# bfGraph/STGraph

Measured on NVIDIA B200. Metric: gcn_fused_aggregation_fwd_bwd_algorithmic_hbm_gbs, higher is better.
Workload: dtype f32

## Files before the change

include/stgraph_b200.h:

```cpp
#ifndef STGRAPH_B200_H_
#define STGRAPH_B200_H_

#include <stddef.h>
#include <stdint.h>

#ifdef __cplusplus
extern "C" {
#endif

#define STG_ABI_VERSION 3

typedef enum StgStatus {
  STG_OK = 0,
  STG_ERR_INVALID_ARGUMENT = -1,
  STG_ERR_CUDA = -2,
  STG_ERR_UNSUPPORTED = -3,
  STG_ERR_WORKSPACE_TOO_SMALL = -4,
  STG_ERR_CAPACITY = -5
} StgStatus;

typedef struct StgCsrView {
  const int32_t* row_offset;
  const int32_t* column_indices;
  const int32_t* eids;
  const int32_t* node_ids;
  int32_t num_nodes;
  int32_t num_edges;
  int32_t eid_base;
  int32_t eids_identity;
  const int32_t* hub_rows;
  const int32_t* hub_count;
  int32_t hub_threshold;
  int32_t hub_capacity;
  int32_t* work_queue;
} StgCsrView;

int stg_abi_version(void);
const char* stg_last_error(void);
int stg_device_info(int device, int32_t* sm_count, int64_t* l2_bytes, int32_t* cc_major, int32_t* cc_minor);

int stg_agg_scaled_sum_f32(const StgCsrView* g, const float* x, int32_t feat,
                           const float* nbr_scale, const float* edge_scale,
                           const float* row_scale, float* out, void* stream);

typedef struct StgEdgeMeta {
  int32_t col;
  float scale;
} StgEdgeMeta;

int stg_csr_pack_edge_meta_f32(const StgCsrView* g, const float* nbr_scale, const float* edge_scale,
                               StgEdgeMeta* meta, void* stream);

int stg_agg_packed_sum_f32(const StgCsrView* g, const StgEdgeMeta* meta, const float* x, int32_t feat,
                           const float* row_scale, float* out, int32_t accumulate, void* stream);

int stg_agg_packed_sum_strided_f32(const StgCsrView* g, const StgEdgeMeta* meta, const float* x, int32_t feat,
                                   int32_t x_ld, const float* row_scale, float* out, int32_t out_ld,
                                   int32_t accumulate, void* stream);

int stg_agg_scaled_sum_accum_f32(const StgCsrView* g, const float* x, int32_t feat, const float* nbr_scale,
                                 const float* edge_scale, const float* row_scale, float* out, void* stream);

int stg_agg_scaled_sum_red_f32(const StgCsrView* g, const float* x, int32_t feat, const float* nbr_scale,
                               const float* edge_scale, const float* row_scale, float* out, void* stream);

int stg_agg_scaled_sum_rows_f32(const StgCsrView* g, const int32_t* out_rows, const float* x, int32_t feat,
                                const float* nbr_scale, const float* edge_scale, const float* row_scale, float* out,
                                int32_t accumulate, void* stream);

int stg_agg_packed_sum_rows_f32(const StgCsrView* g, const StgEdgeMeta* meta, const int32_t* out_rows, const float* x,
                                int32_t feat, const float* row_scale, float* out, int32_t accumulate, void* stream);

#define STG_MAX_PARTS 16
int stg_agg_scaled_sum_parts_f32(const StgCsrView* g, const float* const* x_parts, const int32_t* part_bounds,
                                 int32_t num_parts, int32_t feat, const float* nbr_scale, const float* edge_scale,
                                 const float* row_scale, float* out, void* stream);

int stg_halo_pull_f32(const float* const* x_parts, const int32_t* part_bounds, int32_t num_parts, const int64_t* ids,
                      int64_t n_ids, int32_t feat, float* out, int32_t max_blocks, void* stream);

int stg_halo_push_f32(const float* own, int32_t feat, const int64_t* send_rows, const int32_t* send_peer,
                      const int64_t* send_slot, int64_t n_items, float* const* peer_halo, int32_t num_parts,
                      int32_t max_blocks, void* stream);

int stg_rows_gather_f32(const float* own, int32_t feat, const int64_t* rows, int64_t n, float* buf, int32_t max_blocks,
                        void* stream);
int stg_halo_send_f32(const float* send_buf, int32_t feat, int32_t num_parts, int32_t my_rank, const int64_t* send_off,
                      float* const* peer_dst, void* stream);
int stg_halo_exchange_f32(const float* own, int32_t feat, const int64_t* send_rows, const int64_t* send_off,
                          float* send_buf, float* const* peer_dst, int32_t* const* peer_flags, const int32_t* seq_values,
                          int32_t value, int32_t num_parts, int32_t my_rank, int32_t gather_blocks, void* stream);
int stg_peer_signal(int32_t* const* peer_flags, int32_t num_parts, int32_t my_rank, int32_t value, void* stream);
// ... 136 lines not shown
```

stgraph_b200/_lib.py:

```python
from __future__ import annotations

import ctypes
import os
import subprocess
from ctypes import POINTER, Structure, c_char_p, c_float, c_int32, c_int64, c_size_t, c_void_p

_HERE = os.path.dirname(os.path.abspath(__file__))
LIB_PATH = os.environ.get("STG_B200_LIB") or os.path.join(_HERE, "lib", "libstgraph_b200.so")
CSRC_DIR = os.path.join(_HERE, "csrc")

ABI_VERSION = 3
VM_MAX_TENSORS = 24
VM_MAX_INSTR = 96
VM_MAX_REGS = 48
VM_MAX_ACC = 8


class StgCsrView(Structure):

    _fields_ = [
        ("row_offset", c_void_p),
        ("column_indices", c_void_p),
        ("eids", c_void_p),
        ("node_ids", c_void_p),
# ... 55 lines not shown
                                                  c_void_p, c_void_p], True),
    "stg_agg_scaled_sum_rows_f32": (ctypes.c_int, [_P(StgCsrView), c_void_p, c_void_p, c_int32, c_void_p, c_void_p, c_void_p,
                                                   c_void_p, c_int32, c_void_p], True),
    "stg_csr_pack_edge_meta_f32": (ctypes.c_int, [_P(StgCsrView), c_void_p, c_void_p, c_void_p, c_void_p], True),
    "stg_agg_packed_sum_f32": (ctypes.c_int, [_P(StgCsrView), c_void_p, c_void_p, c_int32, c_void_p, c_void_p, c_int32,
                                              c_void_p], True),
    "stg_agg_packed_sum_strided_f32": (ctypes.c_int, [_P(StgCsrView), c_void_p, c_void_p, c_int32, c_int32, c_void_p,
                                                      c_void_p, c_int32, c_int32, c_void_p], True),
    "stg_halo_push_f32": (ctypes.c_int, [c_void_p, c_int32, c_void_p, c_void_p, c_void_p, c_int64, _P(c_void_p), c_int32,
                                         c_int32, c_void_p], True),
    "stg_agg_packed_sum_rows_f32": (ctypes.c_int, [_P(StgCsrView), c_void_p, c_void_p, c_void_p, c_int32, c_void_p,
                                                   c_void_p, c_int32, c_void_p], True),
    "stg_rows_gather_f32": (ctypes.c_int, [c_void_p, c_int32, c_void_p, c_int64, c_void_p, c_int32, c_void_p], True),
    "stg_halo_send_f32": (ctypes.c_int, [c_void_p, c_int32, c_int32, c_int32, _P(c_int64), _P(c_void_p), c_void_p], True),
    "stg_halo_exchange_f32": (ctypes.c_int, [c_void_p, c_int32, c_void_p, _P(c_int64), c_void_p, _P(c_void_p), _P(c_void_p),
                                              c_void_p, c_int32, c_int32, c_int32, c_int32, c_void_p], True),
    "stg_peer_signal": (ctypes.c_int, [_P(c_void_p), c_int32, c_int32, c_int32, c_void_p], True),
    "stg_peer_wait": (ctypes.c_int, [c_void_p, c_int32, c_int32, c_int32, c_int64, c_void_p, c_void_p], True),
    "stg_agg_scaled_sum_parts_f32": (ctypes.c_int, [_P(StgCsrView), _P(c_void_p), _P(c_int32), c_int32, c_int32, c_void_p,
                                                    c_void_p, c_void_p, c_void_p, c_void_p], True),
    "stg_halo_pull_f32": (ctypes.c_int, [_P(c_void_p), _P(c_int32), c_int32, c_void_p, c_int64, c_int32, c_void_p, c_int32,
                                         c_void_p], True),
    "stg_agg_scaled_sum_f32_host": (ctypes.c_int, [_P(StgCsrView), c_void_p, c_int32, c_void_p, c_void_p, c_void_p,
                                                   c_void_p, c_void_p, c_size_t, c_void_p], True),
    "stg_agg_scaled_sum_f32_host_async": (ctypes.c_int, [_P(StgCsrView), c_void_p, c_int32, c_void_p, c_void_p, c_void_p,
                                                         c_void_p, c_void_p, c_size_t, c_void_p], True),
    "stg_gat_softmax_fwd_f32": (ctypes.c_int, [_P(StgCsrView), c_void_p, c_void_p, c_void_p, c_int32, c_int32,
                                               c_float, c_void_p, c_void_p, c_void_p, c_void_p], True),
    "stg_gat_softmax_bwd_f32": (ctypes.c_int, [_P(StgCsrView), _P(StgCsrView), c_void_p, c_void_p, c_void_p,
                                               c_void_p, c_void_p, c_void_p, c_void_p, c_int32, c_int32, c_float,
                                               c_void_p, c_void_p, c_void_p, c_void_p, c_void_p], True),
    "stg_vm_run_f32": (ctypes.c_int, [_P(StgCsrView), _P(StgVmProgram), _P(c_void_p), c_void_p], True),
    "stg_edge_dot_f32": (ctypes.c_int, [c_void_p, c_int32, c_void_p, c_void_p, c_int64, c_void_p, c_void_p], True),
    "stg_edge_dot_bwd_f32": (ctypes.c_int, [c_void_p, c_int32, c_void_p, c_void_p, c_int64, c_void_p, c_void_p, c_void_p], True),
    "stg_bias_clamp_f32": (ctypes.c_int, [c_void_p, c_void_p, c_int64, c_int32, c_float, c_float, c_void_p], True),
    "stg_clamp_bwd_f32": (ctypes.c_int, [c_void_p, c_void_p, c_void_p, c_int64, c_float, c_float, c_void_p], True),
    "stg_gru_reset_fwd_f32": (ctypes.c_int, [c_void_p, c_void_p, c_void_p, c_int64, c_void_p], True),
    "stg_gru_reset_bwd_f32": (ctypes.c_int, [c_void_p, c_void_p, c_void_p, c_void_p, c_void_p, c_int64, c_void_p], True),
    "stg_gru_update_fwd_f32": (ctypes.c_int, [c_void_p, c_void_p, c_void_p, c_void_p, c_int64, c_void_p], True),
    "stg_gru_update_bwd_f32": (ctypes.c_int, [c_void_p, c_void_p, c_void_p, c_void_p, c_void_p, c_void_p, c_void_p, c_int64,
                                              c_void_p], True),
    "stg_tgcn_reset_fwd_f32": (ctypes.c_int, [c_void_p, c_void_p, c_void_p, c_int64, c_int32, c_void_p], True),
    "stg_tgcn_reset_bwd_f32": (ctypes.c_int, [c_void_p, c_void_p, c_void_p, c_void_p, c_void_p, c_int64, c_int32, c_void_p], True),
    "stg_tgcn_update_fwd_f32": (ctypes.c_int, [c_void_p, c_void_p, c_void_p, c_int64, c_int32, c_void_p], True),
    "stg_tgcn_update_bwd_f32": (ctypes.c_int, [c_void_p, c_void_p, c_void_p, c_void_p, c_void_p, c_int64, c_int32, c_void_p], True),
    "stg_gemm_tn_workspace_bytes": (c_size_t, [c_int64, c_int32, c_int32], False),
    "stg_gemm_tn_f32": (ctypes.c_int, [c_void_p, c_int64, c_void_p, c_int64, c_int64, c_int32, c_int32, c_void_p, c_void_p,
                                       c_void_p, c_size_t, c_void_p], True),
    "stg_csr_build_workspace_bytes": (c_size_t, [c_int64, c_int32], False),
    "stg_csr_build": (ctypes.c_int, [c_void_p, c_void_p, c_int64, c_int32] + [c_void_p] * 12
                      + [c_void_p, c_size_t, c_void_p], True),
    "stg_degree_norm_f32": (ctypes.c_int, [c_void_p, c_int32, c_void_p, c_void_p], True),
    "stg_weighted_row_degree_f32": (ctypes.c_int, [_P(StgCsrView), c_void_p, c_void_p, c_void_p], True),
    "stg_csr_hub_rows": (ctypes.c_int, [c_void_p, c_int32, c_int32, c_void_p, c_int32, c_void_p, c_void_p], True),
    "stg_snapshot_workspace_bytes": (c_size_t, [c_int64], False),
    "stg_snapshot_keys_from_edges": (ctypes.c_int, [c_void_p, c_void_p, c_int64, c_int32, c_void_p, c_void_p, c_void_p,
                                                    c_size_t, c_void_p], True),
    "stg_snapshot_diff": (ctypes.c_int, [c_void_p, c_int64, c_void_p, c_int64, c_void_p, c_void_p, c_void_p, c_size_t,
                                         c_void_p], True),
    "stg_snapshot_apply": (ctypes.c_int, [c_void_p, c_int64, c_void_p, c_int64, c_void_p, c_int64, c_void_p, c_void_p,
                                          c_void_p, c_size_t, c_void_p], True),
    "stg_snapshot_views": (ctypes.c_int, [c_void_p, c_int64, c_int32, c_int32, c_int32] + [c_void_p] * 10
                           + [c_void_p, c_size_t, c_void_p], True),
    "stg_get_array_i32": (ctypes.c_int, [c_void_p, c_int64, c_void_p, c_void_p], True),
}

EXPORTED_SYMBOLS = tuple(_SIGNATURES)

_lib = None


def build(verbose: bool = False) -> str:
    cmd = ["make", "-C", CSRC_DIR, "-j", str(min(8, os.cpu_count() or 1))]
    res = subprocess.run(cmd, stdout=subprocess.PIPE, stderr=subprocess.STDOUT, text=True)
    if verbose or res.returncode != 0:
        print(res.stdout)
    if res.returncode != 0:
        raise RuntimeError("building libstgraph_b200.so failed (see output above)")
    return LIB_PATH


def load():
    global _lib
    if _lib is not None:
        return _lib
    if not os.path.exists(LIB_PATH):
        raise RuntimeError(
            f"{LIB_PATH} is missing: run `python -c 'import __graft_entry__ as g; g.build()'` "
            "(or `make -C stgraph_b200/csrc`). stgraph_b200 has no CPU fallback.")
    lib = ctypes.CDLL(LIB_PATH)
    for name, (restype, argtypes, _) in _SIGNATURES.items():
        fn = getattr(lib, name)
        fn.restype = restype
        fn.argtypes = argtypes
    if lib.stg_abi_version() != ABI_VERSION:
        raise RuntimeError("libstgraph_b200.so ABI version mismatch; rebuild it")
    _lib = lib
    return lib


def call(name: str, *args):
    lib = load()
    rc = getattr(lib, name)(*args)
    if _SIGNATURES[name][2] and rc != 0:
        raise RuntimeError(f"{name} failed ({rc}): {lib.stg_last_error().decode(errors='replace')}")
    return rc
# ... 11 lines not shown
```

stgraph_b200/csrc/agg.cu:

```cuda
#include "common.cuh"

#include <cooperative_groups.h>

#include <algorithm>
#include <cstdlib>

namespace stg {
namespace {

constexpr int kBlockThreads = 256;
constexpr int kHubThreads = 512;

template <int VEC>
__device__ __forceinline__ typename VecT<VEC>::type ld_row(const float* p) {
  using T = typename VecT<VEC>::type;
  return __ldg(reinterpret_cast<const T*>(p));
}
template <int VEC>
__device__ __forceinline__ void st_row(float* p, typename VecT<VEC>::type v) {
  using T = typename VecT<VEC>::type;
  __stcs(reinterpret_cast<T*>(p), v);
}

struct AggParams {
// ... 149 lines not shown
    const int n = min(GROUP, end - base);
    int j = 0;
    for (; j + UNROLL <= n; j += UNROLL) {
      int c[UNROLL];
      float sc[UNROLL];
      T v[UNROLL][NACC];
      fetch_meta(j, c, sc);
#pragma unroll
      for (int u = 0; u < UNROLL; ++u) {
#pragma unroll
        for (int k = 0; k < NACC; ++k) v[u][k] = rows.load(p, c[u], k);
      }
#pragma unroll
      for (int u = 0; u < UNROLL; ++u) {
#pragma unroll
        for (int k = 0; k < NACC; ++k) fma_vec(acc[k], sc[u], v[u][k]);
      }
    }
    if (j < n) {
      int c[UNROLL];
      float sc[UNROLL];
      T v[UNROLL][NACC];
      fetch_meta(j, c, sc);
#pragma unroll
      for (int u = 0; u < UNROLL; ++u) {
#pragma unroll
        for (int k = 0; k < NACC; ++k) {
          if ((j + u) < n) v[u][k] = rows.load(p, c[u], k);
          else zero_vec(v[u][k]);
        }
      }
#pragma unroll
      for (int u = 0; u < UNROLL; ++u) {
#pragma unroll
        for (int k = 0; k < NACC; ++k) fma_vec(acc[k], sc[u], v[u][k]);
      }
    }
    my_c = nx_c;
    my_s = nx_s;
  }
}

template <int VEC, int GROUP, int NACC, int MODE = kPlain>
__device__ __forceinline__ void accumulate_edges(const AggParams& p, int beg, int end, int first_batch,
                                                 int batch_step, int gl, unsigned gmask,
                                                 typename VecT<VEC>::type (&acc)[NACC]) {
  int c;
  float m, s;
  load_col<MODE>(p, beg + first_batch * GROUP, end, gl, c, m);
  load_scale<MODE>(p, beg + first_batch * GROUP, end, gl, c, m, s);
  accumulate_edges<VEC, GROUP, NACC, 0, MODE>(p, beg, end, first_batch, batch_step, gl, gmask, acc, c, s);
}

template <typename T>
__device__ __forceinline__ T shfl_xor_vec(T v, int o);
template <>
__device__ __forceinline__ float shfl_xor_vec<float>(float v, int o) { return __shfl_xor_sync(0xffffffffu, v, o); }
template <>
__device__ __forceinline__ float2 shfl_xor_vec<float2>(float2 v, int o) {
  return make_float2(__shfl_xor_sync(0xffffffffu, v.x, o), __shfl_xor_sync(0xffffffffu, v.y, o));
}
template <>
__device__ __forceinline__ float4 shfl_xor_vec<float4>(float4 v, int o) {
  return make_float4(__shfl_xor_sync(0xffffffffu, v.x, o), __shfl_xor_sync(0xffffffffu, v.y, o),
                     __shfl_xor_sync(0xffffffffu, v.z, o), __shfl_xor_sync(0xffffffffu, v.w, o));
}


__device__ __forceinline__ float4 ldg_row(const float4* p) { return __ldg(p); }

template <int UNROLL, int MODE>
__device__ __forceinline__ void accumulate_edges_pair(const AggParams& p, int beg, int end, int lane, float4& result,
                                                      int my_c, float my_m, float my_s) {
  static_assert(UNROLL % 2 == 0, "two edges per step");
  constexpr int STEPS = UNROLL / 2;
  const int half = lane >> 4;
  const int hl = lane & 15;
  const unsigned ld_bytes = static_cast<unsigned>(p.ld) * 4u;
  const char* base0;
  const char* base1;
  {
    const int last = (p.width - 1) / 4 * 4;
    int o0 = hl * 4, o1 = (hl + 16) * 4;
    if (o0 > last) o0 = last;
    if (o1 > last) o1 = last;
    base0 = reinterpret_cast<const char*>(p.x + o0);
    base1 = reinterpret_cast<const char*>(p.x + o1);
  }
  const bool live1 = (hl + 16) * 4 < p.width;
  auto row0 = [&](int c) { return ldg_row(reinterpret_cast<const float4*>(base0 + static_cast<unsigned long long>(static_cast<unsigned>(c)) * ld_bytes)); };
  auto row1 = [&](int c) {
    float4 v = make_float4(0.f, 0.f, 0.f, 0.f);
    if (live1) v = ldg_row(reinterpret_cast<const float4*>(base1 + static_cast<unsigned long long>(static_cast<unsigned>(c)) * ld_bytes));
    return v;
  };
  float4 acc0 = make_float4(0.f, 0.f, 0.f, 0.f), acc1 = acc0;
  (void)my_m;
  for (int base = beg; base < end; base += 32) {
    int nx_c;
    float nx_m, nx_s;
    load_col<MODE>(p, base + 32, end, lane, nx_c, nx_m);
    load_scale<MODE>(p, base + 32, end, lane, nx_c, nx_m, nx_s);
    const int n = min(32, end - base);
    int j = 0;
    for (; j + UNROLL <= n; j += UNROLL) {
      int c[STEPS];
// ... 188 lines not shown
      if constexpr (PAIR) {
        static_assert(VEC == 4 && GROUP == 32 && NACC == 1, "pair form: one row per warp, float4 lanes");
        accumulate_edges_pair<UNROLL, MODE>(p, beg0, end0, lane, acc[0], c0, 0.f, s0);
      } else {
#pragma unroll
        for (int k = 0; k < NACC; ++k) zero_vec(acc[k]);
        accumulate_edges<VEC, GROUP, NACC, UNROLL, MODE>(p, beg0, end0, 0, 1, gl, gmask, acc, c0, s0);
      }
      write_row<VEC, GROUP, NACC>(p, row0, gl, end0 > beg0, r0, acc, rmw, old);
    }
    slot0 = slot1; row0 = row1; beg0 = beg1; end0 = end1; c0 = c1; s0 = s1; r0 = r1;
    slot1 = slot2; row1 = row2; beg1 = beg2; end1 = end2; c1 = c2; m1 = m2;
    slot2 = slot3; row2 = row3; beg2 = beg3; end2 = end3;
  }
  finish();
}

template <int VEC, int GROUP, int NACC, int MODE, bool PAIR = false>
__global__ void __launch_bounds__(kBlockThreads) agg_rows_kernel(const AggParams p) {
  using T = typename VecT<VEC>::type;
  constexpr int GROUPS_PER_WARP = 32 / GROUP;
  const int lane = threadIdx.x & 31;
  const int gl = lane & (GROUP - 1);
  const unsigned gmask = (GROUP == 32) ? 0xffffffffu : (((1u << GROUP) - 1u) << (lane & ~(GROUP - 1)));
  const int warp = blockIdx.x * (kBlockThreads / 32) + (threadIdx.x >> 5);
  const int row = warp * GROUPS_PER_WARP + lane / GROUP;
  if (row >= p.num_rows) return;
  const int beg = __ldg(p.row_off + row);
  const int end = __ldg(p.row_off + row + 1);
  if (p.hub_threshold > 0 && (end - beg) > p.hub_threshold) return;

  T acc[NACC];
  if constexpr (PAIR) {
    int c;
    float m, s;
    load_col<MODE>(p, beg, end, gl, c, m);
    load_scale<MODE>(p, beg, end, gl, c, m, s);
    accumulate_edges_pair<8, MODE>(p, beg, end, lane, acc[0], c, m, s);
  } else {
#pragma unroll
    for (int k = 0; k < NACC; ++k) zero_vec(acc[k]);
    accumulate_edges<VEC, GROUP, NACC, MODE>(p, beg, end, 0, 1, gl, gmask, acc);
  }

  const int orow = p.out_rows ? __ldg(p.out_rows + row) : row;
  const float r = p.rs ? __ldg(p.rs + orow) : 1.f;
  write_row<VEC, GROUP, NACC>(p, orow, gl, end > beg, r, acc);
  grid_dependency_wait();
}

constexpr int kHubCluster = 8;
constexpr int kClusterRowEdges = 8192;

template <int VEC, int GROUP, int NACC, int MODE>
__global__ void __cluster_dims__(kHubCluster, 1, 1) __launch_bounds__(kHubThreads)
    agg_hub_kernel(const AggParams p) {
  using T = typename VecT<VEC>::type;
  namespace cg = cooperative_groups;
  asm volatile("griddepcontrol.launch_dependents;");
  cg::cluster_group cluster = cg::this_cluster();
  constexpr int GROUPS_PER_WARP = 32 / GROUP;
  constexpr int WARPS = kHubThreads / 32;
  __shared__ T partial[WARPS][GROUP * NACC];
  __shared__ T cta_sum[GROUP * NACC];
  __shared__ int chunk_row[kHubCluster], chunk_beg[kHubCluster], chunk_end[kHubCluster];
  const int lane = threadIdx.x & 31;
  const int wid = threadIdx.x >> 5;
  const int gl = lane & (GROUP - 1);
  const int gidx = lane / GROUP;
  const unsigned gmask = (GROUP == 32) ? 0xffffffffu : (((1u << GROUP) - 1u) << (lane & ~(GROUP - 1)));
  const int crank = static_cast<int>(cluster.block_rank());
  const int cluster_id = blockIdx.x / kHubCluster;
  const int n_clusters = gridDim.x / kHubCluster;
  const int n_hub = min(__ldg(p.hub_count), p.hub_capacity);

  auto cta_partial_sum = [&](int beg, int end, int slot, int slots) {
    T acc[NACC];
#pragma unroll
    for (int k = 0; k < NACC; ++k) zero_vec(acc[k]);
    accumulate_edges<VEC, GROUP, NACC, MODE>(p, beg, end, slot, slots, gl, gmask, acc);
#pragma unroll
    for (int o = GROUP; o < 32; o <<= 1) {
#pragma unroll
      for (int k = 0; k < NACC; ++k) add_vec(acc[k], shfl_xor_vec<T>(acc[k], o));
    }
    if (lane < GROUP) {
#pragma unroll
      for (int k = 0; k < NACC; ++k) partial[wid][k * GROUP + lane] = acc[k];
    }
    __syncthreads();
    if (wid == 0 && lane < GROUP) {
#pragma unroll
      for (int k = 0; k < NACC; ++k) {
        T sum = partial[0][k * GROUP + lane];
        for (int w = 1; w < WARPS; ++w) add_vec(sum, partial[w][k * GROUP + lane]);
        cta_sum[k * GROUP + lane] = sum;
      }
    }
    __syncthreads();
  };
  auto write_hub_row = [&](int row, T (&sum)[NACC]) {
    const int orow = p.out_rows ? __ldg(p.out_rows + row) : row;
    const float r = p.rs ? __ldg(p.rs + orow) : 1.f;
    write_row<VEC, GROUP, NACC>(p, orow, lane, true, r, sum);
  };

  for (int chunk = cluster_id; chunk * kHubCluster < n_hub; chunk += n_clusters) {
    if (threadIdx.x < kHubCluster) {
      const int i = chunk * kHubCluster + threadIdx.x;
      int row = -1, beg = 0, end = 0;
      if (i < n_hub) {
        row = __ldg(p.hub_rows + i);
        beg = __ldg(p.row_off + row);
        end = __ldg(p.row_off + row + 1);
      }
      chunk_row[threadIdx.x] = row;
      chunk_beg[threadIdx.x] = beg;
      chunk_end[threadIdx.x] = end;
    }
    __syncthreads();
    {
      const int row = chunk_row[crank], beg = chunk_beg[crank], end = chunk_end[crank];
      if (row >= 0 && (end - beg) <= kClusterRowEdges) {
        cta_partial_sum(beg, end, wid * GROUPS_PER_WARP + gidx, WARPS * GROUPS_PER_WARP);
        if (wid == 0 && lane < GROUP) {
          T sum[NACC];
#pragma unroll
          for (int k = 0; k < NACC; ++k) sum[k] = cta_sum[k * GROUP + lane];
          write_hub_row(row, sum);
        }
      }
    }
    for (int q = 0; q < kHubCluster; ++q) {
      const int row = chunk_row[q], beg = chunk_beg[q], end = chunk_end[q];
      if (row < 0 || (end - beg) <= kClusterRowEdges) continue;
      cta_partial_sum(beg, end, (crank * WARPS + wid) * GROUPS_PER_WARP + gidx, kHubCluster * WARPS * GROUPS_PER_WARP);
      cluster.sync();
      if (crank == 0 && wid == 0 && lane < GROUP) {
        T sum[NACC];
#pragma unroll
        for (int k = 0; k < NACC; ++k) {
          sum[k] = cta_sum[k * GROUP + lane];
          for (int c = 1; c < kHubCluster; ++c) {
            const T* remote = cluster.map_shared_rank(cta_sum, c);
            add_vec(sum[k], remote[k * GROUP + lane]);
          }
        }
        write_hub_row(row, sum);
      }
      cluster.sync();
    }
    __syncthreads();
  }
}

inline bool pair_mode() {
  static const bool on = [] {
    const char* e = getenv("STG_AGG_PAIR");
    return e == nullptr || e[0] != '0';
  }();
  return on;
}

inline int queue_chunk() {
  static const int v = [] {
    const char* e = getenv("STG_AGG_CHUNK");
    const int c = e ? atoi(e) : 4;
    return c < 0 ? 0 : (c > 4096 ? 4096 : c);
  }();
  return v;
}

inline int hub_grid_mult(int num_edges) {
  static const int v = [] {
    const char* e = getenv("STG_HUB_GRID");
    const int c = e ? atoi(e) : 0;
    return c < 0 ? 0 : (c > 4 ? 4 : c);
  }();
  return v > 0 ? v : (num_edges >= (1 << 24) ? 1 : 2);
}

template <int VEC, int GROUP, int NACC, int MODE>
int launch_agg(const AggParams& p, cudaStream_t stream) {
  constexpr int rows_per_block = (kBlockThreads / 32) * (32 / GROUP);
  const int blocks = (p.num_rows + rows_per_block - 1) / rows_per_block;
  const bool hubs = p.hub_threshold > 0 && p.hub_rows != nullptr;
  const bool overlap = hubs && p.num_edges >= (1 << 18);
  if (hubs) {
    agg_hub_kernel<VEC, GROUP, NACC, MODE><<<hub_grid_mult(p.num_edges) * (sm_count() / kHubCluster) * kHubCluster, kHubThreads, 0, stream>>>(p);
    STG_LAUNCH_CHECK("agg_hub_kernel");
  }
  if (blocks > 0) {
    const bool queue = p.num_rows >= 2 * sm_count() * 4 * (kBlockThreads / 32);
    bool launched = false;
    if constexpr (GROUP == 32 && MODE != kParts) if (queue) {
      launched = true;
      constexpr int MINB = 4;
      constexpr int kRowsPerWarp = 32;
      constexpr int slots_per_block = (kBlockThreads / 32) * kRowsPerWarp;
      const int pblocks = (p.num_rows + slots_per_block - 1) / slots_per_block;
      const bool gq = p.queue != nullptr && queue_chunk() > 0;
      const int gblocks = std::min(sm_count() * MINB, (p.num_rows + 7) / 8);
      if constexpr (VEC == 4 && NACC == 1) {
        if (p.width > 64 && pair_mode()) {
          if (gq) {
            STG_CUDA(launch_overlapped(agg_rows_pipe_kernel<VEC, GROUP, NACC, MINB, 8, MODE, true, true>, gblocks, kBlockThreads,
                                       stream, overlap, p, queue_chunk()));
          } else {
            STG_CUDA(launch_overlapped(agg_rows_pipe_kernel<VEC, GROUP, NACC, MINB, 8, MODE, true>, pblocks, kBlockThreads,
                                       stream, overlap, p, slots_per_block));
          }
          STG_LAUNCH_CHECK("agg_rows_pipe_kernel (pair)");
          return STG_OK;
        }
      }
      if (gq) {
        STG_CUDA(launch_overlapped(agg_rows_pipe_kernel<VEC, GROUP, NACC, MINB, 8 / NACC, MODE, false, true>, gblocks,
                                   kBlockThreads, stream, overlap, p, queue_chunk()));
      } else {
        STG_CUDA(launch_overlapped(agg_rows_pipe_kernel<VEC, GROUP, NACC, MINB, 8 / NACC, MODE>, pblocks, kBlockThreads, stream,
                                   overlap, p, slots_per_block));
      }
    }
    if constexpr (GROUP == 32 && VEC == 4 && NACC == 1 && MODE != kParts) {
      if (!launched && p.width > 64 && pair_mode()) {
        STG_CUDA(launch_overlapped(agg_rows_kernel<VEC, GROUP, NACC, MODE, true>, blocks, kBlockThreads, stream, overlap, p));
        launched = true;
      }
    }
    if (!launched) {
      STG_CUDA(launch_overlapped(agg_rows_kernel<VEC, GROUP, NACC, MODE>, blocks, kBlockThreads, stream, overlap, p));
    }
    STG_LAUNCH_CHECK("agg_rows_kernel");
  }
  return STG_OK;
}

inline bool narrow_vec2() {
  static const bool v = [] {
    const char* e = getenv("STG_AGG_NARROW_VEC2");
    return e ? atoi(e) != 0 : true;
  }();
// ... 65 lines not shown
    al8 = al8 && aligned8(x);
  }
  for (int q = 0; q < nparts; ++q) {
    al16 = al16 && aligned16(parts[q]);
    al8 = al8 && aligned8(parts[q]);
  }
  int vec = 1;
  if (feat % 4 == 0 && p.ld % 4 == 0 && p.ld_out % 4 == 0 && al16) vec = 4;
  else if (feat % 2 == 0 && p.ld % 2 == 0 && p.ld_out % 2 == 0 && al8) vec = 2;
  if (vec == 4 && feat > 32 && feat <= 64 && nparts == 0 && narrow_vec2() && g->work_queue != nullptr &&
      g->num_nodes >= 2 * sm_count() * 4 * (kBlockThreads / 32))
    vec = 2;
  const int chunk = 32 * 4 * vec;
  for (int f0 = 0; f0 < feat; f0 += chunk) {
    p.x = x ? x + f0 : nullptr;
    for (int q = 0; q < nparts; ++q) p.xs[q] = parts[q] + f0;
    p.out = out + f0;
    p.width = min(chunk, feat - f0);
    int rc;
    const int avg_degree = g->num_nodes > 0 ? g->num_edges / g->num_nodes : -1;
    if (nparts > 0) {
      if (vec == 4) rc = dispatch_group<4, kParts>(p, stream, avg_degree);
      else if (vec == 2) rc = dispatch_group<2, kParts>(p, stream, avg_degree);
      else rc = dispatch_group<1, kParts>(p, stream, avg_degree);
    } else if (meta != nullptr) {
      if (vec == 4) rc = dispatch_group<4, kPacked>(p, stream, avg_degree);
      else if (vec == 2) rc = dispatch_group<2, kPacked>(p, stream, avg_degree);
      else rc = dispatch_group<1, kPacked>(p, stream, avg_degree);
    } else {
      if (vec == 4) rc = dispatch_group<4, kPlain>(p, stream, avg_degree);
      else if (vec == 2) rc = dispatch_group<2, kPlain>(p, stream, avg_degree);
      else rc = dispatch_group<1, kPlain>(p, stream, avg_degree);
    }
    if (rc != STG_OK) return rc;
  }
  return STG_OK;
}

}

using namespace stg;

static int validate_view(const StgCsrView* g, bool need_eids) {
  STG_CHECK_ARG(g != nullptr, "graph view is NULL");
  STG_CHECK_ARG(g->num_nodes >= 0 && g->num_edges >= 0, "negative graph size (%d nodes, %d edges)",
                g->num_nodes, g->num_edges);
  STG_CHECK_ARG(g->row_offset != nullptr, "row_offset is NULL");
  STG_CHECK_ARG(g->num_edges == 0 || g->column_indices != nullptr, "column_indices is NULL");
  STG_CHECK_ARG(!need_eids || g->eids_identity || g->num_edges == 0 || g->eids != nullptr,
                "eids is NULL but an edge tensor is indexed by edge id");
  return STG_OK;
}

STG_API int stg_agg_scaled_sum_f32(const StgCsrView* g, const float* x, int32_t feat,
                                      const float* nbr_scale, const float* edge_scale,
                                      const float* row_scale, float* out, void* stream) {
  int rc = validate_view(g, edge_scale != nullptr);
  if (rc != STG_OK) return rc;
  STG_CHECK_ARG(feat > 0, "feat must be positive (got %d)", feat);
  if (g->num_nodes == 0) return STG_OK;
  STG_CHECK_ARG(x != nullptr && out != nullptr, "x / out is NULL");
  STG_CHECK_ARG(x != out, "x and out must not alias");
  return agg_scaled_sum_device(g, x, feat, nbr_scale, edge_scale, row_scale, out, as_stream(stream));
}

static int agg_host_enqueue(const StgCsrView* g, const float* x_host, int32_t feat, const float* nbr_scale_host,
                            const float* edge_scale_host, const float* row_scale_host, float* out_host,
                            void* dev_scratch, size_t dev_scratch_bytes, void* stream, bool synchronize) {
  int rc = validate_view(g, edge_scale_host != nullptr);
  if (rc != STG_OK) return rc;
  STG_CHECK_ARG(feat > 0, "feat must be positive (got %d)", feat);
  if (g->num_nodes == 0) return STG_OK;
  STG_CHECK_ARG(x_host && out_host && dev_scratch, "host buffers / scratch must not be NULL");
  const size_t n = static_cast<size_t>(g->num_nodes), e = static_cast<size_t>(g->num_edges);
  const size_t nf = align_up(n * feat, 4), n4 = align_up(n, 4), e4 = align_up(e, 4);
  const size_t need = (2 * nf + 2 * n4 + e4) * sizeof(float);
  if (dev_scratch_bytes < need) {
    set_error("device scratch too small: %zu bytes given, %zu needed", dev_scratch_bytes, need);
    return STG_ERR_WORKSPACE_TOO_SMALL;
  }
  cudaStream_t s = as_stream(stream);
  float* dx = static_cast<float*>(dev_scratch);
  float* dout = dx + nf;
  float* dns = dout + nf;
  float* drs = dns + n4;
  float* des = drs + n4;
  STG_CUDA(cudaMemcpyAsync(dx, x_host, n * feat * sizeof(float), cudaMemcpyHostToDevice, s));
  if (nbr_scale_host) STG_CUDA(cudaMemcpyAsync(dns, nbr_scale_host, n * sizeof(float), cudaMemcpyHostToDevice, s));
  if (row_scale_host) STG_CUDA(cudaMemcpyAsync(drs, row_scale_host, n * sizeof(float), cudaMemcpyHostToDevice, s));
  if (edge_scale_host) STG_CUDA(cudaMemcpyAsync(des, edge_scale_host, e * sizeof(float), cudaMemcpyHostToDevice, s));
  rc = agg_scaled_sum_device(g, dx, feat, nbr_scale_host ? dns : nullptr, edge_scale_host ? des : nullptr,
                             row_scale_host ? drs : nullptr, dout, s);
  if (rc != STG_OK) return rc;
  STG_CUDA(cudaMemcpyAsync(out_host, dout, n * feat * sizeof(float), cudaMemcpyDeviceToHost, s));
  if (synchronize) STG_CUDA(cudaStreamSynchronize(s));
  return STG_OK;
}

STG_API int stg_agg_scaled_sum_f32_host(const StgCsrView* g, const float* x_host, int32_t feat,
                                        const float* nbr_scale_host, const float* edge_scale_host,
                                        const float* row_scale_host, float* out_host,
                                        void* dev_scratch, size_t dev_scratch_bytes, void* stream) {
  return agg_host_enqueue(g, x_host, feat, nbr_scale_host, edge_scale_host, row_scale_host, out_host, dev_scratch,
                          dev_scratch_bytes, stream, true);
}

// ... 122 lines not shown
```

stgraph_b200/csrc/structure.cu:

```cuda
#include "common.cuh"

#include <cub/device/device_radix_sort.cuh>

namespace stg {
namespace {

constexpr int kThreads = 256;

inline int blocks_for(int64_t n, int per_block = kThreads) {
  int64_t b = (n + per_block - 1) / per_block;
  if (b < 1) b = 1;
  return static_cast<int>(b);
}

__global__ void pack_fwd_keys(const int32_t* __restrict__ src, const int32_t* __restrict__ dst, int64_t n,
                              uint64_t* __restrict__ keys, int32_t* __restrict__ vals) {
  for (int64_t i = blockIdx.x * (int64_t)blockDim.x + threadIdx.x; i < n; i += (int64_t)gridDim.x * blockDim.x) {
    keys[i] = (static_cast<uint64_t>(static_cast<uint32_t>(dst[i])) << 32) | static_cast<uint32_t>(src[i]);
    vals[i] = static_cast<int32_t>(i);
  }
}

__global__ void unpack_sorted(const uint64_t* __restrict__ keys, int64_t n, int32_t num_nodes,
                              int32_t* __restrict__ col, int32_t* __restrict__ eids_identity,
// ... 13 lines not shown
  }
}

__global__ void fill_i32(int32_t* __restrict__ p, int64_t n, int32_t v) {
  for (int64_t i = blockIdx.x * (int64_t)blockDim.x + threadIdx.x; i < n; i += (int64_t)gridDim.x * blockDim.x) p[i] = v;
}

__global__ void pack_bwd_keys(const uint64_t* __restrict__ fwd_keys, int64_t n, uint64_t* __restrict__ keys,
                              int32_t* __restrict__ vals) {
  for (int64_t i = blockIdx.x * (int64_t)blockDim.x + threadIdx.x; i < n; i += (int64_t)gridDim.x * blockDim.x) {
    const uint64_t k = fwd_keys[i];
    keys[i] = (k << 32) | (k >> 32);
    vals[i] = static_cast<int32_t>(i);
  }
}

__global__ void degrees_from_offsets(const int32_t* __restrict__ row_offset, int32_t n, int32_t* __restrict__ deg,
                                     uint32_t* __restrict__ sort_key, int32_t* __restrict__ ids) {
  for (int32_t i = blockIdx.x * blockDim.x + threadIdx.x; i < n; i += gridDim.x * blockDim.x) {
    const int32_t d = row_offset[i + 1] - row_offset[i];
    if (deg) deg[i] = d;
    if (sort_key) sort_key[i] = 0x7fffffffu - static_cast<uint32_t>(d);
    if (ids) ids[i] = i;
  }
}

__global__ void degree_norm_kernel(const int32_t* __restrict__ deg, int32_t n, float* __restrict__ norm) {
  for (int32_t i = blockIdx.x * blockDim.x + threadIdx.x; i < n; i += gridDim.x * blockDim.x) {
    const int32_t d = deg[i];
    norm[i] = d > 0 ? 1.0f / sqrtf(static_cast<float>(d)) : 0.f;
  }
}

__global__ void weighted_row_degree_kernel(const int32_t* __restrict__ row_offset, const int32_t* __restrict__ eids,
                                           int eids_identity, int eid_base, int32_t n,
                                           const float* __restrict__ w, float* __restrict__ out) {
  for (int32_t r = blockIdx.x * blockDim.x + threadIdx.x; r < n; r += gridDim.x * blockDim.x) {
    float acc = 0.f;
    const int32_t e0 = row_offset[r], e1 = row_offset[r + 1];
    for (int32_t e = e0; e < e1; ++e) {
      const int32_t eid = eids_identity ? e : eids[e] - eid_base;
      acc = __fadd_rn(acc, w[eid]);
    }
    out[r] = acc;
  }
}

__global__ void hub_rows_kernel(const int32_t* __restrict__ row_offset, int32_t n, int32_t threshold,
                                int32_t* __restrict__ hub_rows, int32_t capacity, int32_t* __restrict__ hub_count) {
  for (int32_t r = blockIdx.x * blockDim.x + threadIdx.x; r < n; r += gridDim.x * blockDim.x) {
    if (row_offset[r + 1] - row_offset[r] > threshold) {
      const int32_t slot = atomicAdd(hub_count, 1);
      if (slot < capacity) hub_rows[slot] = r;
    }
  }
}

int bits_for(uint32_t max_value) {
  int b = 1;
  while (b < 32 && (max_value >> b) != 0) ++b;
  return b;
}

struct BuildWorkspace {
  uint64_t *keys_a, *keys_b;
  int32_t *vals_a, *vals_b;
  uint32_t *nk_a, *nk_b;
  int32_t *ni_a;
  void* cub_temp;
  size_t cub_bytes;
  size_t total;
};

size_t cub_temp_bytes(int64_t e, int32_t n) {
  size_t a = 0, b = 0;
  cub::DeviceRadixSort::SortPairs(nullptr, a, (const uint64_t*)nullptr, (uint64_t*)nullptr, (const int32_t*)nullptr,
                                  (int32_t*)nullptr, e > 0 ? e : 1, 0, 64, (cudaStream_t)0);
  cub::DeviceRadixSort::SortPairs(nullptr, b, (const uint32_t*)nullptr, (uint32_t*)nullptr, (const int32_t*)nullptr,
                                  (int32_t*)nullptr, (int64_t)(n > 0 ? n : 1), 0, 32, (cudaStream_t)0);
  return a > b ? a : b;
}

BuildWorkspace carve(void* base, int64_t e, int32_t n) {
  BuildWorkspace w;
  const size_t e_ = static_cast<size_t>(e > 0 ? e : 1), n_ = static_cast<size_t>(n > 0 ? n : 1);
  char* p = static_cast<char*>(base);
  size_t off = 0;
  auto take = [&](size_t bytes) {
    char* q = p ? p + off : nullptr;
    off += align_up(bytes, 256);
    return q;
  };
  w.keys_a = reinterpret_cast<uint64_t*>(take(8 * e_));
  w.keys_b = reinterpret_cast<uint64_t*>(take(8 * e_));
  w.vals_a = reinterpret_cast<int32_t*>(take(4 * e_));
  w.vals_b = reinterpret_cast<int32_t*>(take(4 * e_));
  w.nk_a = reinterpret_cast<uint32_t*>(take(4 * n_));
  w.nk_b = reinterpret_cast<uint32_t*>(take(4 * n_));
  w.ni_a = reinterpret_cast<int32_t*>(take(4 * n_));
  w.cub_bytes = cub_temp_bytes(e, n);
  w.cub_temp = take(w.cub_bytes);
  w.total = off;
  return w;
}

}
// ... 50 lines not shown
                                                   nullptr);
    STG_LAUNCH_CHECK("unpack_sorted(bwd)");
  }
  if (num_nodes == 0) return STG_OK;
  const int deg_bits = 31;
  for (int dir = 0; dir < 2; ++dir) {
    const int32_t* ro = dir == 0 ? fwd_row_offset : bwd_row_offset;
    int32_t* deg = dir == 0 ? in_degree : out_degree;
    int32_t* ids = dir == 0 ? fwd_node_ids : bwd_node_ids;
    degrees_from_offsets<<<grid_n, kThreads, 0, s>>>(ro, num_nodes, deg, ids ? w.nk_a : nullptr,
                                                     ids ? w.ni_a : nullptr);
    STG_LAUNCH_CHECK("degrees_from_offsets");
    if (ids) {
      size_t tb = w.cub_bytes;
      STG_CUDA(cub::DeviceRadixSort::SortPairs(w.cub_temp, tb, (const uint32_t*)w.nk_a, w.nk_b,
                                               (const int32_t*)w.ni_a, ids, (int64_t)num_nodes, 0, deg_bits, s));
    }
  }
  return STG_OK;
}

STG_API int stg_degree_norm_f32(const int32_t* degree, int32_t num_nodes, float* norm, void* stream) {
  STG_CHECK_ARG(num_nodes >= 0, "negative node count");
  if (num_nodes == 0) return STG_OK;
  STG_CHECK_ARG(degree && norm, "NULL pointer");
  degree_norm_kernel<<<min(blocks_for(num_nodes), 148 * 8), kThreads, 0, as_stream(stream)>>>(degree, num_nodes, norm);
  STG_LAUNCH_CHECK("degree_norm_kernel");
  return STG_OK;
}

STG_API int stg_weighted_row_degree_f32(const StgCsrView* g, const float* edge_weight, float* out, void* stream) {
  STG_CHECK_ARG(g && g->row_offset, "graph view / row_offset is NULL");
  if (g->num_nodes == 0) return STG_OK;
  STG_CHECK_ARG(out != nullptr, "out is NULL");
  STG_CHECK_ARG(g->num_edges == 0 || edge_weight != nullptr, "edge_weight is NULL");
  STG_CHECK_ARG(g->eids_identity || g->num_edges == 0 || g->eids, "eids is NULL");
  weighted_row_degree_kernel<<<min(blocks_for(g->num_nodes), 148 * 8), kThreads, 0, as_stream(stream)>>>(
      g->row_offset, g->eids, g->eids_identity, g->eid_base, g->num_nodes, edge_weight, out);
  STG_LAUNCH_CHECK("weighted_row_degree_kernel");
  return STG_OK;
}

STG_API int stg_csr_hub_rows(const int32_t* row_offset, int32_t num_nodes, int32_t threshold,
                                int32_t* hub_rows, int32_t capacity, int32_t* hub_count, void* stream) {
  STG_CHECK_ARG(num_nodes >= 0 && capacity >= 0 && threshold >= 0, "negative argument");
  STG_CHECK_ARG(hub_count != nullptr, "hub_count is NULL");
  cudaStream_t s = as_stream(stream);
  STG_CUDA(cudaMemsetAsync(hub_count, 0, sizeof(int32_t), s));
  if (num_nodes == 0) return STG_OK;
  STG_CHECK_ARG(row_offset && (hub_rows || capacity == 0), "NULL pointer");
  hub_rows_kernel<<<min(blocks_for(num_nodes), 148 * 8), kThreads, 0, s>>>(row_offset, num_nodes, threshold,
                                                                          hub_rows, capacity, hub_count);
  STG_LAUNCH_CHECK("hub_rows_kernel");
  return STG_OK;
}
```

stgraph_b200/graph/static/csr.py:

```python
from __future__ import annotations

import ctypes
import os

import numpy as np
import torch

from ... import _lib

HUB_THRESHOLD = int(os.environ.get("STG_HUB_THRESHOLD", "1024"))
PACK_META = os.environ.get("STG_PACK_META", "1") != "0"
MAX_META_REPACKS = 16


def _edges_to_device(edge_list, device, num_nodes=None):
    if isinstance(edge_list, tuple) and len(edge_list) == 2 and not np.isscalar(edge_list[0]) \
            and len(np.shape(edge_list[0])) == 1 and len(edge_list[0]) != 2:
        src, dst = edge_list
        src = torch.as_tensor(src)
        dst = torch.as_tensor(dst)
    else:
        if isinstance(edge_list, torch.Tensor):
            e = edge_list
        else:
# ... 102 lines not shown
                  cap, self._hub_count.data_ptr(), _lib.current_stream_ptr())
        self._hub_enabled = True
        self._hub_sync = sync
        if sync:
            self._hub_enabled = int(self._hub_count.item()) > 0
        self._view = None
        self._alt_views = {}

    def view(self) -> _lib.StgCsrView:
        if self._view is None:
            v = _lib.StgCsrView()
            v.row_offset = self.row_offset.data_ptr()
            v.column_indices = self.column_indices.data_ptr()
            v.eids = self.eids.data_ptr() if self.eids is not None else None
            v.node_ids = self.node_ids.data_ptr() if self.node_ids is not None else None
            v.num_nodes = self.num_nodes
            v.num_edges = self.num_edges
            v.eid_base = self.eid_base
            v.eids_identity = 1 if self.eids_identity else 0
            if self._hub_enabled:
                v.hub_rows = self._hub_rows.data_ptr()
                v.hub_count = self._hub_count.data_ptr()
                v.hub_threshold = HUB_THRESHOLD
                v.hub_capacity = int(self._hub_rows.shape[0])
            else:
                v.hub_rows = None
                v.hub_count = None
                v.hub_threshold = 0
                v.hub_capacity = 0
            self._work_queue = torch.zeros(2, dtype=torch.int32, device=self.row_offset.device)
            v.work_queue = self._work_queue.data_ptr()
            self._view = v
        return self._view


def _alt_view(self, threshold: int) -> _lib.StgCsrView:
    threshold = int(threshold)
    if threshold <= 0 or threshold == HUB_THRESHOLD:
        return self.view()
    alt = getattr(self, "_alt_views", None)
    if alt is None:
        alt = self._alt_views = {}
    if threshold not in alt:
        base = self.view()
        n, e = self.num_nodes, self.num_edges
        cap = e // threshold + 1
        dev = self.row_offset.device
        rows = torch.empty(cap, dtype=torch.int32, device=dev)
        count = torch.zeros(1, dtype=torch.int32, device=dev)
        _lib.call("stg_csr_hub_rows", self.row_offset.data_ptr(), n, threshold, rows.data_ptr(), cap, count.data_ptr(),
                  _lib.current_stream_ptr())
        enabled = True
        if getattr(self, "_hub_sync", False):
            cnt = min(int(count.item()), cap)
            enabled = cnt > 0
            if cnt > 1:
                r = rows[:cnt].long()
                length = (self.row_offset[r + 1] - self.row_offset[r]).long()
                order = torch.sort(length * self.num_nodes + (self.num_nodes - 1 - r), descending=True).indices
                rows[:cnt] = rows[:cnt][order]
        v = _lib.StgCsrView()
        for name, _ in _lib.StgCsrView._fields_:
            setattr(v, name, getattr(base, name))
        v.hub_rows = rows.data_ptr() if enabled else None
        v.hub_count = count.data_ptr() if enabled else None
        v.hub_threshold = threshold if enabled else 0
        v.hub_capacity = cap if enabled else 0
        alt[threshold] = (v, rows, count)
    return alt[threshold][0]


CSR.view_with_hub_threshold = _alt_view


def build_csr_pair(src: torch.Tensor, dst: torch.Tensor, num_nodes: int, want_perm: bool = False):
    assert src.is_cuda and dst.is_cuda, "stgraph_b200 builds graphs on the GPU only (no CPU fallback)"
    dev = src.device
    e = int(src.shape[0])
    n = int(num_nodes)
    i32 = dict(dtype=torch.int32, device=dev)
    f_ro = torch.empty(n + 1, **i32)
    f_col = torch.empty(e, **i32)
    f_eid = torch.empty(e, **i32)
    f_nid = torch.empty(n, **i32)
    b_ro = torch.empty(n + 1, **i32)
    b_col = torch.empty(e, **i32)
    b_eid = torch.empty(e, **i32)
    b_nid = torch.empty(n, **i32)
    in_deg = torch.empty(n, **i32)
    out_deg = torch.empty(n, **i32)
    perm = torch.empty(e, **i32) if want_perm else None
    n_unique = torch.zeros(1, **i32)
    ws_bytes = _lib.load().stg_csr_build_workspace_bytes(e, n)
    ws = torch.empty(ws_bytes, dtype=torch.uint8, device=dev)
    _lib.call("stg_csr_build", src.data_ptr(), dst.data_ptr(), e, n,
              f_ro.data_ptr(), f_col.data_ptr(), f_eid.data_ptr(), f_nid.data_ptr(),
              b_ro.data_ptr(), b_col.data_ptr(), b_eid.data_ptr(), b_nid.data_ptr(),
              in_deg.data_ptr(), out_deg.data_ptr(), _lib.ptr(perm), n_unique.data_ptr(),
              ws.data_ptr(), ws_bytes, _lib.current_stream_ptr())
    fwd = CSR(f_ro, f_col, f_eid, f_nid, in_deg, out_deg, eid_base=0, eids_identity=True)
    bwd = CSR(b_ro, b_col, b_eid, b_nid, out_deg, in_deg, eid_base=0, eids_identity=False)
    return fwd, bwd, perm, n_unique


def get_array(ptr: int, size: int):
    out = (ctypes.c_int32 * size)()
    _lib.call("stg_get_array_i32", ptr, size, ctypes.addressof(out), _lib.current_stream_ptr())
    return list(out)
```

Measured before the change: 994.1.

## Add cp.async shared-memory ring for hub rows and size hub grid from work

The hub aggregation kernel now prefetches gathered float4 neighbor rows into a dynamic shared-memory ring with cp.async, keeping several loads in flight per thread. For large graphs it also counts hub edges on device and lets surplus clusters exit early, matching cluster count to hub work instead of a fixed grid multiplier. Hub rows are sorted by degree on the GPU with a bitonic kernel, replacing the host-side torch sort. The changes add shared-memory pressure and a per-launch reduction over hub rows, which may reduce occupancy or add latency.

```diff
diff --git a/include/stgraph_b200.h b/include/stgraph_b200.h
--- a/include/stgraph_b200.h
+++ b/include/stgraph_b200.h
@@ -38,6 +38,7 @@
 int stg_abi_version(void);
 const char* stg_last_error(void);
 int stg_device_info(int device, int32_t* sm_count, int64_t* l2_bytes, int32_t* cc_major, int32_t* cc_minor);
+int stg_agg_set_hub_clusters(int32_t clusters);
 
 int stg_agg_scaled_sum_f32(const StgCsrView* g, const float* x, int32_t feat,
                            const float* nbr_scale, const float* edge_scale,
diff --git a/stgraph_b200/_lib.py b/stgraph_b200/_lib.py
--- a/stgraph_b200/_lib.py
+++ b/stgraph_b200/_lib.py
@@ -131,6 +131,7 @@
                       + [c_void_p, c_size_t, c_void_p], True),
     "stg_degree_norm_f32": (ctypes.c_int, [c_void_p, c_int32, c_void_p, c_void_p], True),
     "stg_weighted_row_degree_f32": (ctypes.c_int, [_P(StgCsrView), c_void_p, c_void_p, c_void_p], True),
+    "stg_agg_set_hub_clusters": (ctypes.c_int, [c_int32], True),
     "stg_csr_hub_rows": (ctypes.c_int, [c_void_p, c_int32, c_int32, c_void_p, c_int32, c_void_p, c_void_p], True),
     "stg_snapshot_workspace_bytes": (c_size_t, [c_int64], False),
     "stg_snapshot_keys_from_edges": (ctypes.c_int, [c_void_p, c_void_p, c_int64, c_int32, c_void_p, c_void_p, c_void_p,
diff --git a/stgraph_b200/csrc/agg.cu b/stgraph_b200/csrc/agg.cu
--- a/stgraph_b200/csrc/agg.cu
+++ b/stgraph_b200/csrc/agg.cu
@@ -225,6 +225,85 @@
   accumulate_edges<VEC, GROUP, NACC, 0, MODE>(p, beg, end, first_batch, batch_step, gl, gmask, acc, c, s);
 }
 
+__device__ __forceinline__ void cp_async16(float4* dst, const void* src) {
+  asm volatile("cp.async.cg.shared.global [%0], [%1], 16;" ::"r"(static_cast<unsigned>(__cvta_generic_to_shared(dst))),
+               "l"(src)
+               : "memory");
+}
+__device__ __forceinline__ void cp_async_commit() { asm volatile("cp.async.commit_group;" ::: "memory"); }
+template <int N>
+__device__ __forceinline__ void cp_async_wait() { asm volatile("cp.async.wait_group %0;" ::"n"(N) : "memory"); }
+
+constexpr int kRingChunks = 20;
+template <int GROUP, int NACC>
+__host__ __device__ constexpr int ring_depth() { return GROUP < kRingChunks / NACC ? GROUP : kRingChunks / NACC; }
+
+template <int GROUP, int NACC, int MODE>
+__device__ __forceinline__ void accumulate_edges_ring(const AggParams& p, int beg, int end, int first_batch,
+                                                      int batch_step, int gl, unsigned gmask, float4 (&acc)[NACC],
+                                                      float4* ring) {
+  constexpr int D = ring_depth<GROUP, NACC>();
+  constexpr int UNROLL = (GROUP >= 8 ? 8 : GROUP) / (NACC > 2 ? 2 : 1);
+  static_assert(D <= GROUP, "the ring looks at most one batch ahead");
+  const RowLoader<4, GROUP, NACC, MODE> rows(p, gl);
+  auto issue = [&](int slot, int c) {
+#pragma unroll
+    for (int k = 0; k < NACC; ++k) {
+      if (rows.live[k])
+        cp_async16(ring + (slot * NACC + k) * kHubThreads,
+                   rows.base[k] + static_cast<unsigned long long>(static_cast<unsigned>(c)) * rows.ld_bytes);
+    }
+  };
+  const int stride = batch_step * GROUP;
+  int base = beg + first_batch * GROUP;
+  int c0, c1;
+  float s0, s1, m;
+  load_col<MODE>(p, base, end, gl, c0, m);
+  load_scale<MODE>(p, base, end, gl, c0, m, s0);
+  load_col<MODE>(p, base + stride, end, gl, c1, m);
+  load_scale<MODE>(p, base + stride, end, gl, c1, m, s1);
+  {
+    const int n = min(GROUP, end - base);
+#pragma unroll
+    for (int i = 0; i < D; ++i) {
+      const int c = __shfl_sync(gmask, c0, i, GROUP);
+      if (i < n) issue(i, c);
+      cp_async_commit();
+    }
+  }
+  int t = 0;
+  for (; base < end; base += stride) {
+    int c2;
+    float s2;
+    load_col<MODE>(p, base + 2 * stride, end, gl, c2, m);
+    load_scale<MODE>(p, base + 2 * stride, end, gl, c2, m, s2);
+    const int n = min(GROUP, end - base);
+    const int n1 = min(GROUP, end - base - stride);
+    for (int j = 0; j < n; ++j) {
+      cp_async_wait<D - 1>();
+      const float sc = __shfl_sync(gmask, s0, j, GROUP);
+#pragma unroll
+      for (int k = 0; k < NACC; ++k) {
+        float4 v = make_float4(0.f, 0.f, 0.f, 0.f);
+        if (rows.live[k]) v = ring[(t * NACC + k) * kHubThreads];
+        fma_vec(acc[k], sc, v);
+      }
+      const int jj = j + D;
+      const int c = __shfl_sync(gmask, jj < GROUP ? c0 : c1, jj & (GROUP - 1), GROUP);
+      if (jj < GROUP ? jj < n : jj - GROUP < n1) issue(t, c);
+      cp_async_commit();
+      t = t + 1 == D ? 0 : t + 1;
+    }
+    if (n % UNROLL != 0) {
+#pragma unroll
+      for (int k = 0; k < NACC; ++k) fma_vec(acc[k], 0.f, make_float4(0.f, 0.f, 0.f, 0.f));
+    }
+    c0 = c1; s0 = s1;
+    c1 = c2; s1 = s2;
+  }
+  cp_async_wait<0>();
+}
+
 template <typename T>
 __device__ __forceinline__ T shfl_xor_vec(T v, int o);
 template <>
@@ -519,18 +598,30 @@
 constexpr int kHubCluster = 8;
 constexpr int kClusterRowEdges = 8192;
 
+constexpr int kHubEdgeCost = 4;
+
+__device__ __forceinline__ int hub_clusters_for(long long hub_edges, long long num_edges, int max_clusters) {
+  const long long rest = num_edges - hub_edges > 0 ? num_edges - hub_edges : 1;
+  const long long sms = (hub_edges * kHubEdgeCost * max_clusters * kHubCluster + rest - 1) / rest;
+  const long long c = (sms + kHubCluster - 1) / kHubCluster;
+  return static_cast<int>(c < 1 ? 1 : (c > max_clusters ? max_clusters : c));
+}
+
 template <int VEC, int GROUP, int NACC, int MODE>
 __global__ void __cluster_dims__(kHubCluster, 1, 1) __launch_bounds__(kHubThreads)
-    agg_hub_kernel(const AggParams p) {
+    agg_hub_kernel(const AggParams p, int size_from_work) {
   using T = typename VecT<VEC>::type;
   namespace cg = cooperative_groups;
   asm volatile("griddepcontrol.launch_dependents;");
   cg::cluster_group cluster = cg::this_cluster();
   constexpr int GROUPS_PER_WARP = 32 / GROUP;
   constexpr int WARPS = kHubThreads / 32;
+  constexpr bool kRing = VEC == 4 && MODE != kParts;
+  extern __shared__ float4 ring[];
   __shared__ T partial[WARPS][GROUP * NACC];
   __shared__ T cta_sum[GROUP * NACC];
   __shared__ int chunk_row[kHubCluster], chunk_beg[kHubCluster], chunk_end[kHubCluster];
+  __shared__ unsigned long long hub_edges;
   const int lane = threadIdx.x & 31;
   const int wid = threadIdx.x >> 5;
   const int gl = lane & (GROUP - 1);
@@ -538,14 +629,29 @@
   const unsigned gmask = (GROUP == 32) ? 0xffffffffu : (((1u << GROUP) - 1u) << (lane & ~(GROUP - 1)));
   const int crank = static_cast<int>(cluster.block_rank());
   const int cluster_id = blockIdx.x / kHubCluster;
-  const int n_clusters = gridDim.x / kHubCluster;
+  int n_clusters = gridDim.x / kHubCluster;
   const int n_hub = min(__ldg(p.hub_count), p.hub_capacity);
+
+  if (size_from_work) {
+    if (threadIdx.x == 0) hub_edges = 0;
+    __syncthreads();
+    unsigned long long e = 0;
+    for (int i = threadIdx.x; i < n_hub; i += kHubThreads) {
+      const int r = __ldg(p.hub_rows + i);
+      e += static_cast<unsigned>(__ldg(p.row_off + r + 1) - __ldg(p.row_off + r));
+    }
+    atomicAdd(&hub_edges, e);
+    __syncthreads();
+    n_clusters = hub_clusters_for(static_cast<long long>(hub_edges), p.num_edges, n_clusters);
+    if (cluster_id >= n_clusters) return;
+  }
 
   auto cta_partial_sum = [&](int beg, int end, int slot, int slots) {
     T acc[NACC];
 #pragma unroll
     for (int k = 0; k < NACC; ++k) zero_vec(acc[k]);
-    accumulate_edges<VEC, GROUP, NACC, MODE>(p, beg, end, slot, slots, gl, gmask, acc);
+    if constexpr (kRing) accumulate_edges_ring<GROUP, NACC, MODE>(p, beg, end, slot, slots, gl, gmask, acc, ring + threadIdx.x);
+    else accumulate_edges<VEC, GROUP, NACC, MODE>(p, beg, end, slot, slots, gl, gmask, acc);
 #pragma unroll
     for (int o = GROUP; o < 32; o <<= 1) {
 #pragma unroll
@@ -638,14 +744,7 @@
   return v;
 }
 
-inline int hub_grid_mult(int num_edges) {
-  static const int v = [] {
-    const char* e = getenv("STG_HUB_GRID");
-    const int c = e ? atoi(e) : 0;
-    return c < 0 ? 0 : (c > 4 ? 4 : c);
-  }();
-  return v > 0 ? v : (num_edges >= (1 << 24) ? 1 : 2);
-}
+int g_hub_clusters = 0;
 
 template <int VEC, int GROUP, int NACC, int MODE>
 int launch_agg(const AggParams& p, cudaStream_t stream) {
@@ -654,7 +753,21 @@
   const bool hubs = p.hub_threshold > 0 && p.hub_rows != nullptr;
   const bool overlap = hubs && p.num_edges >= (1 << 18);
   if (hubs) {
-    agg_hub_kernel<VEC, GROUP, NACC, MODE><<<hub_grid_mult(p.num_edges) * (sm_count() / kHubCluster) * kHubCluster, kHubThreads, 0, stream>>>(p);
+    constexpr bool kRing = VEC == 4 && MODE != kParts;
+    constexpr int ring_bytes = kRing ? ring_depth<GROUP, NACC>() * NACC * kHubThreads * 16 : 0;
+    auto kernel = agg_hub_kernel<VEC, GROUP, NACC, MODE>;
+    static const cudaError_t attr = cudaFuncSetAttribute(kernel, cudaFuncAttributeMaxDynamicSharedMemorySize, ring_bytes);
+    STG_CUDA(attr);
+    const int max_clusters = sm_count() / kHubCluster;
+    int clusters = kRing ? max_clusters : 2 * max_clusters;
+    int size_from_work = 0;
+    if (g_hub_clusters > 0) {
+      clusters = std::min(g_hub_clusters, max_clusters);
+    } else if (p.num_edges >= (1 << 24)) {
+      clusters = max_clusters;
+      size_from_work = 1;
+    }
+    kernel<<<clusters * kHubCluster, kHubThreads, ring_bytes, stream>>>(p, size_from_work);
     STG_LAUNCH_CHECK("agg_hub_kernel");
   }
   if (blocks > 0) {
@@ -826,6 +939,12 @@
   return STG_OK;
 }
 
+STG_API int stg_agg_set_hub_clusters(int32_t clusters) {
+  STG_CHECK_ARG(clusters >= 0, "clusters must be >= 0 (got %d)", clusters);
+  g_hub_clusters = clusters;
+  return STG_OK;
+}
+
 STG_API int stg_agg_scaled_sum_f32(const StgCsrView* g, const float* x, int32_t feat,
                                       const float* nbr_scale, const float* edge_scale,
                                       const float* row_scale, float* out, void* stream) {
diff --git a/stgraph_b200/csrc/structure.cu b/stgraph_b200/csrc/structure.cu
--- a/stgraph_b200/csrc/structure.cu
+++ b/stgraph_b200/csrc/structure.cu
@@ -89,6 +89,34 @@
     if (row_offset[r + 1] - row_offset[r] > threshold) {
       const int32_t slot = atomicAdd(hub_count, 1);
       if (slot < capacity) hub_rows[slot] = r;
+    }
+  }
+}
+
+__global__ void __launch_bounds__(1024) sort_hub_rows_kernel(const int32_t* __restrict__ row_offset,
+                                                             int32_t* __restrict__ hub_rows, int32_t capacity,
+                                                             const int32_t* __restrict__ hub_count) {
+  const int n = min(*hub_count, capacity);
+  int pow2 = 1;
+  while (pow2 < n) pow2 <<= 1;
+  auto first = [&](int a, int b) {
+    const int da = row_offset[a + 1] - row_offset[a], db = row_offset[b + 1] - row_offset[b];
+    return da > db || (da == db && a < b);
+  };
+  for (int k = 2; k <= pow2; k <<= 1) {
+    for (int j = k >> 1; j > 0; j >>= 1) {
+      for (int i = threadIdx.x; i < pow2 / 2; i += blockDim.x) {
+        const int lo = (i / j) * 2 * j + i % j;
+        const int hi = j == k / 2 ? (i / j) * 2 * j + 2 * j - 1 - i % j : lo + j;
+        if (hi < n) {
+          const int a = hub_rows[lo], b = hub_rows[hi];
+          if (first(b, a)) {
+            hub_rows[lo] = b;
+            hub_rows[hi] = a;
+          }
+        }
+      }
+      __syncthreads();
     }
   }
 }
@@ -245,5 +273,9 @@
   hub_rows_kernel<<<min(blocks_for(num_nodes), 148 * 8), kThreads, 0, s>>>(row_offset, num_nodes, threshold,
                                                                           hub_rows, capacity, hub_count);
   STG_LAUNCH_CHECK("hub_rows_kernel");
-  return STG_OK;
-}
+  if (capacity > 1) {
+    sort_hub_rows_kernel<<<1, 1024, 0, s>>>(row_offset, hub_rows, capacity, hub_count);
+    STG_LAUNCH_CHECK("sort_hub_rows_kernel");
+  }
+  return STG_OK;
+}
diff --git a/stgraph_b200/graph/static/csr.py b/stgraph_b200/graph/static/csr.py
--- a/stgraph_b200/graph/static/csr.py
+++ b/stgraph_b200/graph/static/csr.py
@@ -178,13 +178,7 @@
                   _lib.current_stream_ptr())
         enabled = True
         if getattr(self, "_hub_sync", False):
-            cnt = min(int(count.item()), cap)
-            enabled = cnt > 0
-            if cnt > 1:
-                r = rows[:cnt].long()
-                length = (self.row_offset[r + 1] - self.row_offset[r]).long()
-                order = torch.sort(length * self.num_nodes + (self.num_nodes - 1 - r), descending=True).indices
-                rows[:cnt] = rows[:cnt][order]
+            enabled = int(count.item()) > 0
         v = _lib.StgCsrView()
         for name, _ in _lib.StgCsrView._fields_:
             setattr(v, name, getattr(base, name))
```

After: 984.1 (median of 6 runs). No clear change (-1.0%).
